# RobotSail/2048-PPO

Measured on AMD Instinct MI355X. Metric: env-steps/sec (whole node) at 65536 parallel 4x4 boards, 1/2/4/8 MI355X, higher is better.
Workload: dtype int8

## Files before the change

2048-ppo_amd/csrc/env_rollout.hip:

```cpp
#include <hip/hip_runtime.h>
#include <stdint.h>

#include <atomic>
#include <type_traits>

#include "board.hpp"
#include "rowtable.hpp"
#include "line11_lds.hpp"
#include "step.hpp"
#include "rollout_step.hpp"
#include "launch_util.hpp"
#include "../../include/g2048.h"

using namespace g2048;

namespace {

__device__ __forceinline__ uint4 fresh_from_words(const uint4 &r, uint32_t &p1, uint32_t &v1, uint32_t &p2,
                                                  uint32_t &v2) {
    p1 = r.x >> 28;
    v1 = r.y < kTwoThreshold ? 1u : 2u;
    const uint32_t k2 = (uint32_t)(((uint64_t)r.z * 15u) >> 32);
    p2 = k2 + (k2 >= p1 ? 1u : 0u);
    v2 = r.w < kTwoThreshold ? 1u : 2u;
// ... 42 lines not shown
template <int kAddr, bool kWide>
__global__ __launch_bounds__(1024) void env_rollout_kernel(uint4 *__restrict__ boards, int64_t n, int64_t steps,
                                                           uint4 *__restrict__ tb, uint8_t *__restrict__ ta,
                                                           int32_t *__restrict__ tp, uint32_t *__restrict__ tpot,
                                                           uint8_t *__restrict__ tf, RngArgs rng,
                                                           uint32_t *__restrict__ ticket) {
    __shared__ __attribute__((aligned(16))) uint32_t s_row[kRolloutLdsWords];
    i32x4 fa{};
    if constexpr (kAddr != kAddrValu) fa = line_mfma_frag();
    stage_row_table(s_row);
    if constexpr (kAddr != kAddrValu) asm volatile("" : "+v"(fa));
    const uint64_t ctr0 = rng_counter(rng);
    const int64_t stride = (int64_t)gridDim.x * blockDim.x;
    for (int64_t i = (int64_t)blockIdx.x * blockDim.x + threadIdx.x; i < n; i += stride) {
        RolloutLane s;
        s.b = boards[i];
        const uint32_t env = rng.env_base + (uint32_t)i;
        const uint32_t li = (uint32_t)i;
        s.legal = legal_mask(s.b);
        if (s.legal == 0u) {
            uint32_t p1, v1, p2, v2;
            s.b = fresh_from_words(philox_draw(rng.seed, ctr0 + (uint64_t)steps, env, 2u), p1, v1, p2, v2);
            MonoStats ms;
            s.legal = fresh_stats(p1, v1, p2, v2, ms);
            s.S = carry_pack(ms);
        } else {
            s.S = carry_pack(mono_stats(s.b));
        }
        s.empt_b = emptiness(s.b);
        uint64_t pair = ctr0 >> 1;
        s.D = philox_draw(rng.seed, pair, env, 1u);
        s.ph = philox_start(rng.seed, pair + 1u, env, 1u);
        fresh_prep(s, s_row);
        refill_lines<kAddr>(s, s_row, s.S >> 24, fa);
        using Rows = std::conditional_t<kWide, TrajRows, TrajRowsNarrow>;
        Rows tr = Rows::at(tb, ta, tp, tpot, tf, li);
        uint64_t left = (uint64_t)steps;
        if ((ctr0 & 1u) && left > 0u) {
            philox_rounds<0, 5>(s.ph);
            rollout_step<true, false, true, kAddr, Rows>(s, s_row, tr, rng.seed, pair + 2u, env, fa);
            tr.next(n);
            pair++;
            left--;
        }
        for (uint64_t pairs = left >> 1; pairs != 0u; pairs--, pair++) {
            if (__all(s.S < ((kFastPairMax + 1u) << 24))) {
                rollout_step<false, true, true, kAddr, Rows>(s, s_row, tr, rng.seed, pair + 2u, env, fa);
                tr.next(n);
                rollout_step<true, true, true, kAddr, Rows>(s, s_row, tr, rng.seed, pair + 2u, env, fa);
            } else {
                rollout_step<false, false, true, kAddr, Rows>(s, s_row, tr, rng.seed, pair + 2u, env, fa);
                tr.next(n);
                rollout_step<true, false, true, kAddr, Rows>(s, s_row, tr, rng.seed, pair + 2u, env, fa);
            }
            tr.next(n);
        }
        if (left & 1u) rollout_step<false, false, true, kAddr, Rows>(s, s_row, tr, rng.seed, pair + 2u, env, fa);
        boards[i] = s.b;
    }
    if (ticket) {
        __syncthreads();
        if (threadIdx.x == 0 &&
            __hip_atomic_fetch_add(ticket, 1u, __ATOMIC_RELAXED, __HIP_MEMORY_SCOPE_AGENT) == gridDim.x - 1u) {
            __hip_atomic_fetch_add(const_cast<uint64_t *>(rng.counter_dev), (uint64_t)steps, __ATOMIC_RELAXED,
                                   __HIP_MEMORY_SCOPE_AGENT);
            __hip_atomic_store(ticket, 0u, __ATOMIC_RELAXED, __HIP_MEMORY_SCOPE_AGENT);
        }
// ... 64 lines not shown
```

2048-ppo_amd/csrc/line11_lds.hpp:

```cpp
#pragma once
#include <hip/hip_runtime.h>
#include <stdint.h>

#include "board.hpp"
#include "rowtable.hpp"

namespace {

__device__ const g2048::lut::Line11Table kLine11 __attribute__((aligned(16))) = g2048::lut::Line11Table();
static_assert(g2048::lut::line11_table_ok(g2048::lut::Line11Table()), "kLine11 fields against slide_entry / line_entry");

__device__ const g2048::lut::FreshTable kFresh __attribute__((aligned(16))) = g2048::lut::FreshTable();
__device__ const g2048::lut::FreshLineTable kFreshLines __attribute__((aligned(16))) = g2048::lut::FreshLineTable();
static_assert(g2048::lut::fresh_lines_ok(g2048::lut::FreshTable(), g2048::lut::FreshLineTable()), "kFreshLines against the kFresh boards");
constexpr uint32_t kLineLdsBytes = g2048::lut::kFusedEntriesPadded * 8u;
constexpr uint32_t kFreshBoardBase = kLineLdsBytes;
constexpr uint32_t kFreshLineBase = kFreshBoardBase + g2048::lut::kFreshEntries * 16u;
constexpr uint32_t kFreshStatBase = kFreshLineBase + g2048::lut::kFreshEntries * 16u;
constexpr uint32_t kRolloutLdsWords = (kFreshStatBase + 4096u) / 4u;
static_assert(kRolloutLdsWords * 4u <= 160u * 1024u, "the tables fit the 160 KiB of LDS");
constexpr uint32_t kMaxLineDigit = g2048::lut::kLineBase - 1u;
static_assert(8u * g2048::lut::line11_index(kMaxLineDigit, kMaxLineDigit, kMaxLineDigit, kMaxLineDigit) + 8u <= g2048::lut::kFusedEntries * 8u &&
              g2048::lut::kFusedEntries * 8u <= kLineLdsBytes, "kLine11 reads stay inside the table");
static_assert(g2048::lut::line11_index(kMaxLineDigit, kMaxLineDigit, kMaxLineDigit, kMaxLineDigit) < 65536u, "column indices fit the packed-u16 sums");

typedef uint16_t u16x2 __attribute__((ext_vector_type(2)));
__device__ __forceinline__ u16x2 as_u16x2(uint32_t x) { return __builtin_bit_cast(u16x2, x); }

__device__ __forceinline__ void line11_addrs(const uint4 &b, uint32_t (&ra)[4], uint32_t (&ca)[4]) {
    const u16x2 k02 = {8, 968}, k13 = {88, 10648};
    const uint32_t w[4] = {b.x, b.y, b.z, b.w};
    u16x2 A[4], B[4];
#pragma unroll
    for (int i = 0; i < 4; i++) {
        A[i] = as_u16x2(__builtin_amdgcn_perm(0u, w[i], 0x0C020C00u));
        B[i] = as_u16x2(__builtin_amdgcn_perm(0u, w[i], 0x0C030C01u));
        ra[i] = __builtin_amdgcn_udot2(B[i], k13, __builtin_amdgcn_udot2(A[i], k02, 0u, false), false);
    }
    const u16x2 c02 = A[0] + A[1] * (u16x2){11, 11} + A[2] * (u16x2){121, 121} + A[3] * (u16x2){1331, 1331};
    const u16x2 c13 = B[0] + B[1] * (u16x2){11, 11} + B[2] * (u16x2){121, 121} + B[3] * (u16x2){1331, 1331};
    const uint32_t p02 = __builtin_bit_cast(uint32_t, c02), p13 = __builtin_bit_cast(uint32_t, c13);
    ca[0] = (p02 & 0xFFFFu) << 3;
    ca[1] = (p13 & 0xFFFFu) << 3;
    ca[2] = (p02 >> 16) << 3;
    ca[3] = (p13 >> 16) << 3;
}

typedef int i32x4 __attribute__((ext_vector_type(4)));
typedef int i32x16 __attribute__((ext_vector_type(16)));
constexpr uint32_t kLineHiScale = 8u * g2048::lut::kLineBase * g2048::lut::kLineBase;
constexpr int line_mfma_weight(uint32_t q, uint32_t c) {
    const uint32_t line = q & 7u, r = c >> 2, col = c & 3u;
    const uint32_t pos = line < 4u ? (r == line ? col : 4u) : (col == line - 4u ? r : 4u);
// ... 43 lines not shown
                const uint32_t lo_c = (uint32_t)line_mfma_model(t, h ? other : mine, h ? mine : other, h, 4u + r);
                const uint32_t hi_c = (uint32_t)line_mfma_model(t, h ? other : mine, h ? mine : other, h, 12u + r);
                if (lo_r > 960u || hi_r > 120u || lo_c > 960u || hi_c > 120u) return false;
                if (lo_r + kLineHiScale * hi_r != 8u * g2048::lut::line11_index(c[4 * r], c[4 * r + 1], c[4 * r + 2], c[4 * r + 3])) return false;
                if (lo_c + kLineHiScale * hi_c != 8u * g2048::lut::line11_index(c[r], c[4 + r], c[8 + r], c[12 + r])) return false;
            }
        }
    return true;
}
static_assert(line_mfma_weights_int8(), "the MFMA address weights fit int8");
static_assert(line_mfma_ok(), "the MFMA address model against line11_index");
__device__ const LineMfmaTable kLineMfmaA __attribute__((aligned(16))) = LineMfmaTable();
__device__ __forceinline__ i32x4 line_mfma_frag() {
    return *reinterpret_cast<const i32x4 *>(kLineMfmaA.a[threadIdx.x & 63u]);
}
__device__ __forceinline__ i32x16 line11_limbs_mfma(const uint4 &b, const i32x4 &fa) {
    const i32x4 bv = {(int)b.x, (int)b.y, (int)b.z, (int)b.w};
    const i32x16 zero = {0, 0, 0, 0, 0, 0, 0, 0, 0, 0, 0, 0, 0, 0, 0, 0};
    return __builtin_amdgcn_mfma_i32_32x32x32_i8(fa, bv, zero, 0, 0, 0);
}
__device__ __forceinline__ void line11_addrs_from_limbs(const i32x16 &d, uint32_t (&ra)[4], uint32_t (&ca)[4]) {
#pragma unroll
    for (int i = 0; i < 4; i++) {
        ra[i] = __umul24((uint32_t)d[8 + i], kLineHiScale) + (uint32_t)d[i];
        ca[i] = __umul24((uint32_t)d[12 + i], kLineHiScale) + (uint32_t)d[4 + i];
    }
}
__device__ __forceinline__ void line11_addrs_mfma(const uint4 &b, const i32x4 &fa, uint32_t (&ra)[4], uint32_t (&ca)[4]) {
    line11_addrs_from_limbs(line11_limbs_mfma(b, fa), ra, ca);
}
__device__ __forceinline__ uint2 lds_rec(const uint32_t *tab, uint32_t addr) {
    return *reinterpret_cast<const uint2 *>(reinterpret_cast<const char *>(tab) + addr);
}
__device__ __forceinline__ uint32_t lds_half(const uint32_t *tab, uint32_t addr) {
    return *reinterpret_cast<const uint16_t *>(reinterpret_cast<const char *>(tab) + addr);
}

constexpr uint32_t kUnpackStartSel = 0x05010400u;
constexpr uint32_t kUnpackEndSel = 0x07030602u;

constexpr uint32_t kPackRowsSel = 0x05040100u;
constexpr uint32_t kPackColsSel = 0x05010400u;
constexpr uint32_t kPackEndAdd = 0x02020202u;
constexpr uint32_t perm_model(uint32_t hi, uint32_t lo, uint32_t sel) {
    const uint64_t src = ((uint64_t)hi << 32) | lo;
    uint32_t r = 0u;
    for (uint32_t j = 0u; j < 4u; j++) {
        const uint32_t s = (sel >> (8u * j)) & 0xFFu;
        r |= (s < 8u ? (uint32_t)(src >> (8u * s)) & 0xFFu : 0u) << (8u * j);
    }
    return r;
}
struct Rows4 {
    uint32_t x, y, z, w;
};
constexpr Rows4 orient_rows_model(uint32_t e0, uint32_t e1, uint32_t e2, uint32_t e3, bool vert, bool rev) {
    const uint32_t psel = (vert ? kPackColsSel : kPackRowsSel) + (rev ? kPackEndAdd : 0u);
    const uint32_t x02 = perm_model(e2, e0, psel), x13 = perm_model(e3, e1, psel);
    const uint32_t xl02 = x02 & 0x0F0F0F0Fu, xh02 = (x02 >> 4) & 0x0F0F0F0Fu;
    const uint32_t xl13 = x13 & 0x0F0F0F0Fu, xh13 = (x13 >> 4) & 0x0F0F0F0Fu;
    const uint32_t pA = vert ? xl13 : xh02, pB = vert ? xh02 : xl13;
    return Rows4{perm_model(pA, xl02, kUnpackStartSel), perm_model(xh13, pB, kUnpackStartSel),
                 perm_model(pA, xl02, kUnpackEndSel), perm_model(xh13, pB, kUnpackEndSel)};
}
constexpr Rows4 unpack_transpose_model(uint32_t e0, uint32_t e1, uint32_t e2, uint32_t e3, bool vert, bool rev) {
    const uint32_t usel = rev ? kUnpackEndSel : kUnpackStartSel;
    const uint32_t w[4] = {perm_model(e0 >> 4, e0, usel) & 0x0F0F0F0Fu, perm_model(e1 >> 4, e1, usel) & 0x0F0F0F0Fu,
                           perm_model(e2 >> 4, e2, usel) & 0x0F0F0F0Fu, perm_model(e3 >> 4, e3, usel) & 0x0F0F0F0Fu};
    const uint32_t p = perm_model(w[1], w[0], 0x05010400u), q = perm_model(w[1], w[0], 0x07030602u);
    const uint32_t u = perm_model(w[3], w[2], 0x05010400u), v = perm_model(w[3], w[2], 0x07030602u);
    if (!vert) return Rows4{w[0], w[1], w[2], w[3]};
    return Rows4{perm_model(u, p, 0x05040100u), perm_model(u, p, 0x07060302u), perm_model(v, q, 0x05040100u),
                 perm_model(v, q, 0x07060302u)};
}
constexpr bool orient_rows_ok() {
    for (uint32_t k = 0u; k < 11u; k++) {
        uint32_t e[4] = {0u, 0u, 0u, 0u};
        for (uint32_t i = 0u; i < 4u; i++)
            for (uint32_t j = 0u; j < 8u; j++) e[i] |= ((k + 3u * j + 5u * i) % 11u) << (4u * j);
        for (uint32_t o = 0u; o < 4u; o++) {
            const Rows4 n = orient_rows_model(e[0], e[1], e[2], e[3], (o & 2u) != 0u, (o & 1u) != 0u);
            const Rows4 r = unpack_transpose_model(e[0], e[1], e[2], e[3], (o & 2u) != 0u, (o & 1u) != 0u);
            if (n.x != r.x || n.y != r.y || n.z != r.z || n.w != r.w) return false;
        }
    }
    return true;
}
static_assert(orient_rows_ok(), "the orientation network against unpack_row, transpose and sel4");
__device__ __forceinline__ uint4 orient_rows(uint32_t e0, uint32_t e1, uint32_t e2, uint32_t e3, uint32_t psel, bool vert) {
    const uint32_t x02 = __builtin_amdgcn_perm(e2, e0, psel), x13 = __builtin_amdgcn_perm(e3, e1, psel);
    const uint32_t xl02 = x02 & 0x0F0F0F0Fu, xh02 = (x02 >> 4) & 0x0F0F0F0Fu;
    const uint32_t xl13 = x13 & 0x0F0F0F0Fu, xh13 = (x13 >> 4) & 0x0F0F0F0Fu;
    const uint32_t pA = vert ? xl13 : xh02, pB = vert ? xh02 : xl13;
    return make_uint4(__builtin_amdgcn_perm(pA, xl02, kUnpackStartSel), __builtin_amdgcn_perm(xh13, pB, kUnpackStartSel),
                      __builtin_amdgcn_perm(pA, xl02, kUnpackEndSel), __builtin_amdgcn_perm(xh13, pB, kUnpackEndSel));
}

typedef __attribute__((address_space(3))) void lds_void_t;
typedef __attribute__((address_space(1))) void glb_void_t;
__device__ __forceinline__ void stage_row_table(uint32_t *s_row) {
    constexpr int kLinePieces = (int)(kLineLdsBytes / 1024u);
    constexpr int kFreshPieces = (int)(g2048::lut::kFreshEntries * 16u / 1024u);
    static_assert(kLineLdsBytes % 1024u == 0u && g2048::lut::kFreshEntries * 16u % 1024u == 0u, "whole 1 KiB pieces");
    static_assert(sizeof(kLine11.v) == kLineLdsBytes && sizeof(kFresh.b) == kFreshPieces * 1024 &&
                  sizeof(kFreshLines.a) == kFreshPieces * 1024 && sizeof(kFresh.st) == 4096, "table sizes");
    constexpr int kAll = kLinePieces + 2 * kFreshPieces + 4;
    static_assert(kAll * 1024 == (int)(kRolloutLdsWords * 4u), "the pieces fill the allocation");
    const char *src = reinterpret_cast<const char *>(kLine11.v);
    const char *src2 = reinterpret_cast<const char *>(kFresh.b);
    const char *src3 = reinterpret_cast<const char *>(kFreshLines.a);
    const char *src4 = reinterpret_cast<const char *>(kFresh.st);
    char *dst = reinterpret_cast<char *>(s_row);
    const int lane = threadIdx.x & 63, wave = threadIdx.x >> 6, nw = blockDim.x >> 6;
    for (int c = wave; c < kAll; c += nw) {
        const char *g;
        if (c < kLinePieces) g = src + 1024 * c;
        else if (c < kLinePieces + kFreshPieces) g = src2 + 1024 * (c - kLinePieces);
        else if (c < kLinePieces + 2 * kFreshPieces) g = src3 + 1024 * (c - kLinePieces - kFreshPieces);
        else g = src4 + 1024 * (c - kLinePieces - 2 * kFreshPieces);
        __builtin_amdgcn_global_load_lds((glb_void_t *)(g + 16 * lane), (lds_void_t *)(dst + 1024 * c), 16, 0, 0);
    }
    __builtin_amdgcn_s_waitcnt(0);
    __syncthreads();
}

}
```

2048-ppo_amd/csrc/mc_search.hip:

```cpp
#include <hip/hip_runtime.h>
#include <stdint.h>

#include "board.hpp"
#include "rowtable.hpp"
#include "line11_lds.hpp"
#include "step.hpp"
#include "rollout_step.hpp"
#include "launch_util.hpp"
#include "../../include/g2048.h"

using namespace g2048;

namespace {

constexpr int64_t kMaxPlayouts = 4096, kMaxDepth = 65536;

__device__ __forceinline__ void mc_playout(RolloutLane &s, const uint32_t *__restrict__ tab, uint64_t seed, uint64_t c,
                                           uint32_t env, int depth) {
    refill_lines(s, tab, s.M);
    const TrajRows none{};
    uint64_t pair = c >> 1;
    s.D = philox_draw(seed, pair, env, 1u);
    s.ph = philox_start(seed, pair + 1u, env, 1u);
    int t = 0;
    if (c & 1u) {
        philox_rounds<0, 5>(s.ph);
        rollout_step<true, false, false>(s, tab, none, seed, pair + 2u, env);
        pair++;
        t = 1;
    }
    for (; s.legal != 0u && t + 2 <= depth; t += 2, pair++) {
        if (__all(s.M <= kFastPairMax)) {
            rollout_step<false, true, false>(s, tab, none, seed, pair + 2u, env);
            if (s.legal == 0u) break;
            rollout_step<true, true, false>(s, tab, none, seed, pair + 2u, env);
        } else {
            rollout_step<false, false, false>(s, tab, none, seed, pair + 2u, env);
            if (s.legal == 0u) break;
            rollout_step<true, false, false>(s, tab, none, seed, pair + 2u, env);
        }
    }
    if (s.legal != 0u && t < depth) rollout_step<false, false, false>(s, tab, none, seed, pair + 2u, env);
}

__global__ __launch_bounds__(1024) void mc_search_kernel(const uint4 *__restrict__ boards, uint32_t total,
                                                         uint32_t playouts, int depth, RngArgs rng,
                                                         unsigned long long *__restrict__ score_sum,
                                                         unsigned long long *__restrict__ move_sum,
                                                         uint8_t *__restrict__ legal_out, uint8_t *__restrict__ best_out,
                                                         uint32_t *__restrict__ arrived) {
    __shared__ __attribute__((aligned(16))) uint32_t s_row[kRolloutLdsWords];
    stage_row_table(s_row);
    const uint64_t ctr0 = rng_counter(rng);
    const uint32_t lane = threadIdx.x & 63u;
    const uint32_t stride = gridDim.x * blockDim.x;
    for (uint32_t L0 = blockIdx.x * blockDim.x + (threadIdx.x & ~63u); L0 < total; L0 += stride) {
        const uint32_t L = L0 + lane;
        const bool valid = L < total;
        uint32_t g = 0xFFFFFFFFu, p = 0u;
        uint32_t score = 0u, moves = 0u;
        if (valid) {
            g = L / playouts;
            p = L - g * playouts;
            const uint4 root = boards[g >> 2];
            uint32_t pts0, mx0;
            uint4 moved = apply_move(root, g & 3u, pts0, mx0);
            if (!eq4(moved, root)) {
                const uint32_t env = rng.env_base + L;
                const uint4 ph = philox_draw(rng.seed, ctr0, env, 0u);
                spawn<G2048_RNG_PHILOX>(moved, ph.x, ph.y, nullptr, rng, (int64_t)L);
                RolloutLane s;
                s.b = moved;
                s.legal = legal_mask(moved);
                s.M = board_max(moved);
                s.score = pts0;
                s.moves = 0u;
                if (s.legal != 0u && depth > 0) mc_playout(s, s_row, rng.seed, ctr0, env, depth);
                score = s.score;
                moves = s.moves;
            }
        }
        unsigned long long sc = score;
        uint32_t mv = moves;
#pragma unroll
        for (uint32_t off = 1u; off < 64u; off <<= 1) {
// ... 85 lines not shown
```

2048-ppo_amd/csrc/rollout_step.hpp:

```cpp
#pragma once
#include <hip/hip_runtime.h>
#include <stdint.h>

#include "board.hpp"
#include "rowtable.hpp"
#include "line11_lds.hpp"
#include "step.hpp"

namespace {

using namespace g2048;

constexpr uint32_t kFastPairMax = 8u;
static_assert(kFastPairMax + 1u + 1u <= kMaxLineDigit, "a fast pair (start <= 8) stays inside kLine11");
static_assert(lut::kFreshLineAddrMax + 8u <= kLineLdsBytes, "fresh boards' line records inside kLine11");
static_assert(60u * 15u + 4u * 14u + 3u == lut::kFreshEntries - 1u, "kFresh index range");
static_assert(kFreshStatBase + 4u * lut::kFreshEntries <= kRolloutLdsWords * 4u, "kFresh reads stay inside the allocation");

__device__ __forceinline__ uint32_t mono_value_packed(uint32_t S) {
    const u16x2 m = __builtin_elementwise_max(as_u16x2(S & 0x000F0F00u), as_u16x2((S >> 4) & 0x000F0F00u));
    const uint32_t best256 = __builtin_amdgcn_udot2(m, (u16x2){1, 256}, 0u, false);
    const uint32_t corner = __builtin_amdgcn_ubfe(0x9009u, S, 1u);
    return best256 >> (9u - 2u * corner);
}
__device__ __forceinline__ uint32_t stats_bytes(uint32_t SR, uint32_t SC) {
    return __builtin_amdgcn_perm(SC, SR, 0x0C04000Cu);
}

struct RolloutLane {
    uint4 b;
    uint32_t legal;
    uint32_t M;
    uint32_t S;
    int empt_b;
    uint2 R[4], C[4];
    uint4 D;
    PhiloxState ph;
    uint32_t fbo;
    uint32_t fst;
    uint4 fla;
    uint32_t score;
    uint32_t moves;
};

__device__ __forceinline__ void fresh_prep(RolloutLane &s, const uint32_t *__restrict__ tab) {
    const uint32_t a = s.D.z, bw = s.D.w;
    const uint64_t pb = (uint64_t)bw * 15u;
    const uint32_t k2 = (uint32_t)(pb >> 32);
    const uint32_t i = 60u * (a >> 28) + 4u * k2 + ((a << 4) >= kTwoThreshold ? 2u : 0u) +
                       ((uint32_t)pb >= kTwoThreshold ? 1u : 0u);
    const char *t = reinterpret_cast<const char *>(tab);
    s.fbo = kFreshBoardBase + 16u * i;
    s.fla = *reinterpret_cast<const uint4 *>(t + kFreshLineBase + 16u * i);
    s.fst = *reinterpret_cast<const uint32_t *>(t + kFreshStatBase + 4u * i);
}
__device__ __forceinline__ void reset_reload(RolloutLane &s, const uint32_t *__restrict__ tab) {
    uint4 la = s.fla;
    asm volatile("" : "+v"(la.x), "+v"(la.y), "+v"(la.z), "+v"(la.w));
    s.b = *reinterpret_cast<const uint4 *>(reinterpret_cast<const char *>(tab) + s.fbo);
    s.R[0] = lds_rec(tab, la.x & 0xFFFFu);
    s.R[1] = lds_rec(tab, la.x >> 16);
    s.R[2] = lds_rec(tab, la.y & 0xFFFFu);
    s.R[3] = lds_rec(tab, la.y >> 16);
    s.C[0] = lds_rec(tab, la.z & 0xFFFFu);
    s.C[1] = lds_rec(tab, la.z >> 16);
    s.C[2] = lds_rec(tab, la.w & 0xFFFFu);
    s.C[3] = lds_rec(tab, la.w >> 16);
}

constexpr int kAddrValu = 0, kAddrMfma = 1;

template <int kAddr = kAddrValu>
__device__ __forceinline__ void refill_lines(RolloutLane &s, const uint32_t *__restrict__ tab, uint32_t mx, const i32x4 &fa = i32x4{}) {
    const uint4 ab = sel4(mx > kMaxLineDigit, make_uint4(0u, 0u, 0u, 0u), s.b);
    uint32_t ra[4], ca[4];
    if constexpr (kAddr == kAddrValu) line11_addrs(ab, ra, ca);
    else line11_addrs_mfma(ab, fa, ra, ca);
#pragma unroll
    for (int i = 0; i < 4; i++) {
        s.R[i] = lds_rec(tab, ra[i]);
        s.C[i] = lds_rec(tab, ca[i]);
    }
}

constexpr int kWaitLds = 0xC07F;

struct TrajRows {
    uint4 *b;
    uint8_t *a;
    int32_t *p;
    uint32_t *pot;
    uint8_t *f;
    __device__ __forceinline__ static TrajRows at(uint4 *tb, uint8_t *ta, int32_t *tp, uint32_t *tpot, uint8_t *tf, uint32_t i) {
        return TrajRows{tb + i, ta + i, tp + i, tpot + i, tf + i};
    }
    __device__ __forceinline__ void next(int64_t n) {
        b += n;
        a += n;
        p += n;
        pot += n;
        f += n;
    }
    __device__ __forceinline__ void put_b(const uint4 &v) const { *b = v; }
    __device__ __forceinline__ void put_a(uint32_t v) const { *a = (uint8_t)v; }
    __device__ __forceinline__ void put_p(uint32_t v) const { *p = (int32_t)v; }
    __device__ __forceinline__ void put_pot(uint32_t v) const { *pot = v; }
    __device__ __forceinline__ void put_f(uint32_t v) { *f = (uint8_t)v; }
};
struct TrajRowsNarrow {
    char *b, *a, *p, *pot, *f;
    uint32_t o1, o4, o16;
    __device__ __forceinline__ static TrajRowsNarrow at(uint4 *tb, uint8_t *ta, int32_t *tp, uint32_t *tpot, uint8_t *tf, uint32_t i) {
        return TrajRowsNarrow{(char *)tb, (char *)ta, (char *)tp, (char *)tpot, (char *)tf, i, 4u * i, 16u * i};
    }
    __device__ __forceinline__ void next(int64_t n) {
        const uint32_t n1 = (uint32_t)n;
        o1 += n1;
        o4 += 4u * n1;
        o16 += 16u * n1;
        asm("" : "+v"(o1), "+v"(o4), "+v"(o16));
    }
    __device__ __forceinline__ void put_b(const uint4 &v) const { *reinterpret_cast<uint4 *>(b + o16) = v; }
    __device__ __forceinline__ void put_a(uint32_t v) const { *reinterpret_cast<uint8_t *>(a + o1) = (uint8_t)v; }
    __device__ __forceinline__ void put_p(uint32_t v) const { *reinterpret_cast<int32_t *>(p + o4) = (int32_t)v; }
    __device__ __forceinline__ void put_pot(uint32_t v) const { *reinterpret_cast<uint32_t *>(pot + o4) = v; }
    __device__ __forceinline__ void put_f(uint32_t v) {
        asm("" : "+v"(o1));
        *reinterpret_cast<uint8_t *>(f + o1) = (uint8_t)v;
    }
};

template <bool kOdd, bool kSmall, bool kTraj, int kAddr = kAddrValu, class Rows = TrajRows>
__device__ __forceinline__ void rollout_step(RolloutLane &s, const uint32_t *__restrict__ tab, Rows &tr,
                                             uint64_t seed, uint64_t next_pair, uint32_t env, const i32x4 &fa = i32x4{}) {
    if constexpr (kTraj && (!kOdd || kSmall)) __builtin_amdgcn_s_waitcnt(kWaitLds);
    if constexpr (kTraj) tr.put_b(s.b);
    const uint32_t u = kOdd ? s.D.y : s.D.x;
    const uint64_t pa = (uint64_t)u * (uint32_t)__popc(s.legal);
    const uint32_t a = kth_bit4(s.legal, (uint32_t)(pa >> 32)), r = (uint32_t)pa;
    const bool vert = a < 2u, rev = (a & 1u) != 0u;
    const uint32_t e0 = vert ? s.C[0].x : s.R[0].x, e1 = vert ? s.C[1].x : s.R[1].x;
    const uint32_t e2 = vert ? s.C[2].x : s.R[2].x, e3 = vert ? s.C[3].x : s.R[3].x;
    const uint32_t h0 = vert ? s.C[0].y : s.R[0].y, h1 = vert ? s.C[1].y : s.R[1].y;
    const uint32_t h2 = vert ? s.C[2].y : s.R[2].y, h3 = vert ? s.C[3].y : s.R[3].y;
    const uint32_t mono_b = kTraj ? mono_value_packed(s.S) : 0u;
    const uint32_t pbase = vert ? kPackColsSel : kPackRowsSel;
    const uint32_t psel = rev ? pbase + kPackEndAdd : pbase;
    uint4 moved = orient_rows(e0, e1, e2, e3, psel, vert);
    uint32_t pts = (((h0 >> 16) & 0xFFFu) + ((h1 >> 16) & 0xFFFu) + ((h2 >> 16) & 0xFFFu) + ((h3 >> 16) & 0xFFFu)) << 2;
    uint32_t Ma = __builtin_bit_cast(uint32_t, __builtin_elementwise_max(__builtin_elementwise_max(as_u16x2(h0), as_u16x2(h1)),
                                                                         __builtin_elementwise_max(as_u16x2(h2), as_u16x2(h3)))) >> 28;
    if constexpr (kTraj && kSmall && !kOdd) __builtin_amdgcn_s_waitcnt(kWaitLds);
    if (!kSmall && (kTraj ? s.S >> 24 : s.M) > kMaxLineDigit) {
        uint32_t mx;
        moved = apply_move(s.b, a, pts, mx);
        Ma = board_max(moved);
    }
    const uint32_t rm[4] = {moved.x, moved.y, moved.z, moved.w};
    const uint32_t Zm[4] = {zm(moved.x), zm(moved.y), zm(moved.z), zm(moved.w)};
    uint32_t pos_a = 0u;
    if constexpr (kTraj && kAddr == kAddrValu) pos_a = first_cell_eq(rm, Ma);
    const uint32_t n0 = __popc(Zm[0]), n01 = __popc(Zm[1]) + n0, n012 = __popc(Zm[2]) + n01;
    const uint32_t empt_a = __popc(Zm[3]) + n012;
    const uint64_t prod = (uint64_t)r * empt_a;
    const uint32_t k = (uint32_t)(prod >> 32);
    const uint32_t v = (uint32_t)prod < kTwoThreshold ? 1u : 2u;
    const uint4 pre = moved;
    uint32_t row, col, mr0 = 0u, mr1 = 0u, mc0 = 0u, mc1 = 0u;
    bool r1 = false, r2 = false, r3 = false, c1 = false, c2 = false, c3 = false;
    if constexpr (kTraj) {
        const uint32_t P = n0 | (n01 << 8) | (n012 << 16);
        const uint32_t ger = (__umul24(k, 0x010101u) + (0x808080u - P)) & 0x808080u;
        row = __popc(ger);
        const uint32_t kr = k - __builtin_amdgcn_ubfe(P, 8u * row - 8u, 8u);
        mr0 = (uint32_t)__builtin_amdgcn_sbfe((int)row, 0u, 1u), mr1 = (uint32_t)__builtin_amdgcn_sbfe((int)ger, 15u, 1u);
        asm("" : "+v"(mr0), "+v"(mr1));
        const uint32_t z = pick4m(mr0, mr1, Zm[0], Zm[1], Zm[2], Zm[3]);
        const uint32_t PC = __umul24(z >> 7, 0x010101u);
        const uint32_t gec = (__umul24(kr, 0x010101u) + (0x808080u - PC)) & 0x808080u;
        col = __popc(gec);
        mc0 = (uint32_t)__builtin_amdgcn_sbfe((int)col, 0u, 1u), mc1 = (uint32_t)__builtin_amdgcn_sbfe((int)gec, 15u, 1u);
        asm("" : "+v"(mc0), "+v"(mc1));
        const uint32_t bits = v << (8u * col);
        const uint32_t blo = bop3<~kA & kB>(mr1, bits, 0u), bhi = mr1 & bits;
        moved.x = bop3<kA | (~kB & kC)>(moved.x, mr0, blo);
        moved.y = bop3<kA | (kB & kC)>(moved.y, mr0, blo);
// ... 25 lines not shown
    if constexpr (kAddr == kAddrValu) {
        line11_addrs(ab, ra, ca);
    } else {
        const i32x16 limbs = line11_limbs_mfma(ab, fa);
        if constexpr (kTraj) pos_a = first_cell_eq(rm, Ma);
        line11_addrs_from_limbs(limbs, ra, ca);
    }
    constexpr uint64_t kW11 = 0x299803C800580008ull;
    const uint32_t rq = kTraj ? pick4m(mr0, mr1, ra[0], ra[1], ra[2], ra[3]) : r3 ? ra[3] : r2 ? ra[2] : r1 ? ra[1] : ra[0];
    const uint32_t cq = kTraj ? pick4m(mc0, mc1, ca[0], ca[1], ca[2], ca[3]) : c3 ? ca[3] : c2 ? ca[2] : c1 ? ca[1] : ca[0];
    const uint32_t rp = rq - va * ((uint32_t)(kW11 >> (16u * col)) & 0xFFFFu);
    const uint32_t cp = cq - va * ((uint32_t)(kW11 >> (16u * row)) & 0xFFFFu);
    uint2 R0 = lds_rec(tab, ra[0]), R1 = lds_rec(tab, ra[1]), R2 = lds_rec(tab, ra[2]), R3 = lds_rec(tab, ra[3]);
    uint2 C0 = lds_rec(tab, ca[0]), C1 = lds_rec(tab, ca[1]), C2 = lds_rec(tab, ca[2]), C3 = lds_rec(tab, ca[3]);
    uint32_t fq = 0u, gq = 0u, fp = 0u, gp = 0u;
    if constexpr (kTraj) {
        fq = lds_half(tab, rq + 4u), gq = lds_half(tab, cq + 4u);
        fp = lds_half(tab, rp + 4u), gp = lds_half(tab, cp + 4u);
    }
    asm volatile("" : "+v"(s.ph.c0), "+v"(s.ph.c1), "+v"(s.ph.c2), "+v"(s.ph.c3)::"memory");
    if constexpr (kOdd) philox_rounds<5, 10>(s.ph);
    else philox_rounds<0, 5>(s.ph);
    if constexpr (kTraj)
        asm volatile("" : "+v"(s.ph.c0), "+v"(s.ph.c1), "+v"(s.ph.c2), "+v"(s.ph.c3), "+v"(R0.y), "+v"(R1.y), "+v"(R2.y), "+v"(R3.y),
                          "+v"(C0.y), "+v"(C1.y), "+v"(C2.y), "+v"(C3.y), "+v"(fq), "+v"(gq), "+v"(fp), "+v"(gp));
    else
        asm volatile("" : "+v"(s.ph.c0), "+v"(s.ph.c1), "+v"(s.ph.c2), "+v"(s.ph.c3), "+v"(R0.y), "+v"(R1.y), "+v"(R2.y), "+v"(R3.y),
                          "+v"(C0.y), "+v"(C1.y), "+v"(C2.y), "+v"(C3.y));
    if constexpr (kTraj) {
        tr.put_a(a);
        tr.put_p(pts);
    }
    const uint32_t SR = R0.y + R1.y + R2.y + R3.y, SC = C0.y + C1.y + C2.y + C3.y;
    const uint32_t SRp = SR - fq + fp, SCp = SC - gq + gp;
    const uint32_t nl = __builtin_amdgcn_perm(SR, SC, 0x0C0C0501u);
    s.legal = (__umul24((nl + 0x7777u) & 0x8888u, 0x249u) >> 12) & 15u;
    if (!kSmall && Ma > kMaxLineDigit) s.legal = legal_mask(moved);
    const bool over = s.legal == 0u;
    s.R[0] = R0, s.R[1] = R1, s.R[2] = R2, s.R[3] = R3;
    s.C[0] = C0, s.C[1] = C1, s.C[2] = C2, s.C[3] = C3;
    if constexpr (kTraj) {
        uint32_t sa = stats_bytes(SRp, SCp) | pos_a;
        const uint32_t pos2 = v > Ma ? sp : v == Ma ? min(pos_a, sp) : pos_a;
        uint32_t S = stats_bytes(SR, SC) | pos2 | (max(Ma, v) << 24);
        if (!kSmall && Ma > kMaxLineDigit) {
            const MonoStats ms = mono_stats(pre);
            sa = carry_pack(ms);
            S = carry_pack(mono_add_tile(ms, pre, sp, v));
        }
        const uint32_t mono_a = mono_value_packed(sa);
        tr.put_pot(mono_b | (mono_a << 8) | ((uint32_t)s.empt_b << 16) | (empt_a << 24));
        uint32_t fl = s.legal;
        s.S = S;
        s.empt_b = (int)empt_a - 1;
        if (over) {
            reset_reload(s, tab);
            uint32_t st = s.fst;
            asm volatile("" : "+v"(st));
            s.legal = st >> 28;
            s.S = st & 0x0FFFFFFFu;
            fl = FLAG_DONE | FLAG_RESET | s.legal;
            s.empt_b = 14;
        }
        tr.put_f(fl);
    } else {
        s.M = max(Ma, v);
        s.score += pts;
        s.moves += 1u;
    }
    if constexpr (kOdd) {
        s.D = make_uint4(s.ph.c0, s.ph.c1, s.ph.c2, s.ph.c3);
        s.ph = philox_start(seed, next_pair, env, 1u);
        if constexpr (kTraj) fresh_prep(s, tab);
    }
}

}
```

2048-ppo_amd/csrc/rowtable.hpp:

```cpp
#pragma once
#include <stdint.h>

namespace g2048 {
namespace lut {

constexpr uint32_t kRowBase = 12u;
constexpr uint32_t kRowEntries = kRowBase * kRowBase * kRowBase * kRowBase;

constexpr uint32_t slide_entry(uint32_t idx) {
    uint32_t c[4] = {idx % 12u, idx / 12u % 12u, idx / 144u % 12u, idx / 1728u};
    uint32_t nz[4] = {0u, 0u, 0u, 0u}, n = 0u;
    for (int j = 0; j < 4; j++)
        if (c[j]) nz[n++] = c[j];
    uint32_t out[4] = {0u, 0u, 0u, 0u}, m = 0u, i = 0u, pts = 0u;
    while (i < n) {
        if (i + 1u < n && nz[i] == nz[i + 1u]) {
            out[m++] = nz[i] + 1u;
            pts += 1u << (nz[i] + 1u);
            i += 2u;
        } else {
            out[m++] = nz[i];
            i += 1u;
        }
    }
// ... 8 lines not shown
        for (uint32_t i = 0; i < kRowEntries; i++) v[i] = slide_entry(i);
    }
};

constexpr uint32_t kLineEntriesPadded = 20992u;

constexpr uint16_t line_entry(uint32_t idx) {
    const uint32_t c[4] = {idx % 12u, idx / 12u % 12u, idx / 144u % 12u, idx / 1728u};
    uint32_t lc = 0u, rc = 0u, can0 = 0u, can3 = 0u;
    for (int j = 0; j < 3; j++) {
        const uint32_t a = c[j], b = c[j + 1];
        if (a != 0u && b != 0u) {
            lc += a >= b ? 1u : 0u;
            rc += b >= a ? 1u : 0u;
        }
        if ((a == 0u && b != 0u) || (a != 0u && a == b)) can0 = 1u;
        if ((a != 0u && b == 0u) || (a != 0u && a == b)) can3 = 1u;
    }
    return (uint16_t)(lc | (rc << 4) | (can0 << 8) | (can3 << 12));
}

struct Line12Table {
    uint16_t v[kLineEntriesPadded];
    constexpr Line12Table() : v() {
        for (uint32_t i = 0; i < kRowEntries; i++) v[i] = line_entry(i);
    }
};


constexpr uint32_t kFreshEntries = 16u * 15u * 4u;

struct FreshTable {
    uint32_t b[kFreshEntries * 4];
    uint32_t st[1024];
    constexpr FreshTable() : b(), st() {
        for (uint32_t p1 = 0; p1 < 16u; p1++)
            for (uint32_t k2 = 0; k2 < 15u; k2++)
                for (uint32_t w = 0; w < 4u; w++) {
                    const uint32_t i = 60u * p1 + 4u * k2 + w, p2 = k2 + (k2 >= p1 ? 1u : 0u);
                    const uint32_t v1 = 1u + (w >> 1), v2 = 1u + (w & 1u);
                    uint32_t c[16] = {};
                    c[p1] = v1;
                    c[p2] = v2;
                    for (uint32_t r = 0; r < 4u; r++)
                        b[4u * i + r] = c[4 * r] | (c[4 * r + 1] << 8) | (c[4 * r + 2] << 16) | (c[4 * r + 3] << 24);
                    uint32_t legal = 0u, L = 0u, R = 0u, T = 0u, B = 0u;
                    for (uint32_t r = 0; r < 4u; r++)
                        for (uint32_t j = 0; j < 3u; j++) {
                            const uint32_t x = c[4 * r + j], y = c[4 * r + j + 1];
                            const uint32_t u = c[4 * j + r], d = c[4 * j + 4 + r];
                            if ((x == 0u && y != 0u) || (x != 0u && x == y)) legal |= 4u;
                            if ((x != 0u && y == 0u) || (x != 0u && x == y)) legal |= 8u;
                            if ((u == 0u && d != 0u) || (u != 0u && u == d)) legal |= 1u;
                            if ((u != 0u && d == 0u) || (u != 0u && u == d)) legal |= 2u;
                            if (x != 0u && y != 0u) {
                                L += x >= y ? 1u : 0u;
                                R += y >= x ? 1u : 0u;
                            }
                            if (u != 0u && d != 0u) {
                                T += u >= d ? 1u : 0u;
                                B += d >= u ? 1u : 0u;
                            }
                        }
                    const uint32_t M = v1 > v2 ? v1 : v2;
                    uint32_t pos = 0u;
                    while (c[pos] != M) pos++;
                    st[i] = pos | (L << 8) | (R << 12) | (T << 16) | (B << 20) | (M << 24) | (legal << 28);
                }
    }
};

constexpr uint32_t kLineBase = 11u;
constexpr uint32_t kFusedEntries = kLineBase * kLineBase * kLineBase * kLineBase;
constexpr uint32_t kFusedEntriesPadded = 14720u;

constexpr uint32_t line11_index(uint32_t c0, uint32_t c1, uint32_t c2, uint32_t c3) {
    return c0 + 11u * c1 + 121u * c2 + 1331u * c3;
}
constexpr uint32_t row12_index(uint32_t c0, uint32_t c1, uint32_t c2, uint32_t c3) {
    return c0 + 12u * c1 + 144u * c2 + 1728u * c3;
}
constexpr uint32_t reverse_nibbles16(uint32_t x) {
    return ((x & 0xFu) << 12) | ((x & 0xF0u) << 4) | ((x >> 4) & 0xF0u) | ((x >> 12) & 0xFu);
}

struct Line11Table {
    uint32_t v[kFusedEntriesPadded * 2];
    constexpr Line11Table() : v() {
        for (uint32_t i = 0; i < kFusedEntries; i++) {
            const uint32_t c0 = i % 11u, c1 = i / 11u % 11u, c2 = i / 121u % 11u, c3 = i / 1331u;
            const uint32_t fwd = slide_entry(row12_index(c0, c1, c2, c3));
            const uint32_t bwd = slide_entry(row12_index(c3, c2, c1, c0));
            v[2u * i] = (fwd & 0xFFFFu) | (reverse_nibbles16(bwd & 0xFFFFu) << 16);
            v[2u * i + 1u] = line_entry(row12_index(c0, c1, c2, c3)) | (fwd & 0xFFFF0000u);
        }
    }
};

constexpr bool line11_table_ok(const Line11Table &t) {
    for (uint32_t i = 0; i < kFusedEntries; i++) {
// ... 17 lines not shown
static_assert(kFreshLineAddrMax < 65536u && kFreshLineAddrMax / 8u < kFusedEntries, "kFreshLines addresses");

struct FreshLineTable {
    uint16_t a[kFreshEntries * 8];
    constexpr FreshLineTable() : a() {
        for (uint32_t p1 = 0; p1 < 16u; p1++)
            for (uint32_t k2 = 0; k2 < 15u; k2++)
                for (uint32_t w = 0; w < 4u; w++) {
                    const uint32_t i = 60u * p1 + 4u * k2 + w, p2 = k2 + (k2 >= p1 ? 1u : 0u);
                    uint32_t c[16] = {};
                    c[p1] = 1u + (w >> 1);
                    c[p2] = 1u + (w & 1u);
                    for (uint32_t r = 0; r < 4u; r++) {
                        a[8u * i + r] = (uint16_t)(8u * line11_index(c[4 * r], c[4 * r + 1], c[4 * r + 2], c[4 * r + 3]));
                        a[8u * i + 4u + r] = (uint16_t)(8u * line11_index(c[r], c[4 + r], c[8 + r], c[12 + r]));
                    }
                }
    }
};

constexpr bool fresh_lines_ok(const FreshTable &f, const FreshLineTable &l) {
    for (uint32_t i = 0; i < kFreshEntries; i++) {
        uint32_t c[16] = {};
        for (uint32_t p = 0; p < 16u; p++) c[p] = (f.b[4u * i + p / 4u] >> (8u * (p % 4u))) & 0xFFu;
        for (uint32_t r = 0; r < 4u; r++) {
            if (l.a[8u * i + r] != 8u * line11_index(c[4 * r], c[4 * r + 1], c[4 * r + 2], c[4 * r + 3])) return false;
            if (l.a[8u * i + 4u + r] != 8u * line11_index(c[r], c[4 + r], c[8 + r], c[12 + r])) return false;
            if (l.a[8u * i + r] > kFreshLineAddrMax || l.a[8u * i + 4u + r] > kFreshLineAddrMax) return false;
        }
    }
    return true;
}

}
}
```

Before: 121.6 billion.

## Carry per-orientation line point sums and max in rollout lane state

In the trajectory rollout path, the per-row and per-column point sums and maxima of the line records' high words are now kept in lane state. They are computed once when lines are refilled or updated, instead of being rebuilt from four high words at each move. The high halves of R/C no longer need to be stored, and fresh-board resets load precomputed sums from an enlarged fresh stat table (8 bytes per entry). This costs extra LDS for the stat table and extra register state, and it tightens the large-tile fallback condition. It is meant to cut VALU work and register pressure per step.

After: 123.2 billion (median of 6 runs). 1.3% higher.

```diff
diff --git a/2048-ppo_amd/csrc/env_rollout.hip b/2048-ppo_amd/csrc/env_rollout.hip
--- a/2048-ppo_amd/csrc/env_rollout.hip
+++ b/2048-ppo_amd/csrc/env_rollout.hip
@@ -98,7 +98,7 @@
         s.D = philox_draw(rng.seed, pair, env, 1u);
         s.ph = philox_start(rng.seed, pair + 1u, env, 1u);
         fresh_prep(s, s_row);
-        refill_lines<kAddr>(s, s_row, s.S >> 24, fa);
+        refill_lines<kAddr, true>(s, s_row, s.S >> 24, fa);
         using Rows = std::conditional_t<kWide, TrajRows, TrajRowsNarrow>;
         Rows tr = Rows::at(tb, ta, tp, tpot, tf, li);
         uint64_t left = (uint64_t)steps;
diff --git a/2048-ppo_amd/csrc/line11_lds.hpp b/2048-ppo_amd/csrc/line11_lds.hpp
--- a/2048-ppo_amd/csrc/line11_lds.hpp
+++ b/2048-ppo_amd/csrc/line11_lds.hpp
@@ -13,12 +13,17 @@
 __device__ const g2048::lut::FreshTable kFresh __attribute__((aligned(16))) = g2048::lut::FreshTable();
 __device__ const g2048::lut::FreshLineTable kFreshLines __attribute__((aligned(16))) = g2048::lut::FreshLineTable();
 static_assert(g2048::lut::fresh_lines_ok(g2048::lut::FreshTable(), g2048::lut::FreshLineTable()), "kFreshLines against the kFresh boards");
+static_assert(g2048::lut::fresh_sums_ok(g2048::lut::FreshTable(), g2048::lut::FreshLineTable(), g2048::lut::Line11Table()),
+              "kFresh line sums against the kLine11 records of the kFresh boards");
 constexpr uint32_t kLineLdsBytes = g2048::lut::kFusedEntriesPadded * 8u;
 constexpr uint32_t kFreshBoardBase = kLineLdsBytes;
 constexpr uint32_t kFreshLineBase = kFreshBoardBase + g2048::lut::kFreshEntries * 16u;
 constexpr uint32_t kFreshStatBase = kFreshLineBase + g2048::lut::kFreshEntries * 16u;
-constexpr uint32_t kRolloutLdsWords = (kFreshStatBase + 4096u) / 4u;
+constexpr uint32_t kFreshStatPieces = 8u;
+constexpr uint32_t kRolloutLdsWords = (kFreshStatBase + 1024u * kFreshStatPieces) / 4u;
 static_assert(kRolloutLdsWords * 4u <= 160u * 1024u, "the tables fit the 160 KiB of LDS");
+constexpr uint32_t kSearchStatPieces = 4u;
+constexpr uint32_t kSearchLdsWords = (kFreshStatBase + 1024u * kSearchStatPieces) / 4u;
 constexpr uint32_t kMaxLineDigit = g2048::lut::kLineBase - 1u;
 static_assert(8u * g2048::lut::line11_index(kMaxLineDigit, kMaxLineDigit, kMaxLineDigit, kMaxLineDigit) + 8u <= g2048::lut::kFusedEntries * 8u &&
               g2048::lut::kFusedEntries * 8u <= kLineLdsBytes, "kLine11 reads stay inside the table");
@@ -128,6 +133,9 @@
 __device__ __forceinline__ uint2 lds_rec(const uint32_t *tab, uint32_t addr) {
     return *reinterpret_cast<const uint2 *>(reinterpret_cast<const char *>(tab) + addr);
 }
+__device__ __forceinline__ uint32_t lds_word(const uint32_t *tab, uint32_t addr) {
+    return *reinterpret_cast<const uint32_t *>(reinterpret_cast<const char *>(tab) + addr);
+}
 __device__ __forceinline__ uint32_t lds_half(const uint32_t *tab, uint32_t addr) {
     return *reinterpret_cast<const uint16_t *>(reinterpret_cast<const char *>(tab) + addr);
 }
@@ -194,14 +202,16 @@
 
 typedef __attribute__((address_space(3))) void lds_void_t;
 typedef __attribute__((address_space(1))) void glb_void_t;
+template <uint32_t kStatPieces = kFreshStatPieces>
 __device__ __forceinline__ void stage_row_table(uint32_t *s_row) {
     constexpr int kLinePieces = (int)(kLineLdsBytes / 1024u);
     constexpr int kFreshPieces = (int)(g2048::lut::kFreshEntries * 16u / 1024u);
     static_assert(kLineLdsBytes % 1024u == 0u && g2048::lut::kFreshEntries * 16u % 1024u == 0u, "whole 1 KiB pieces");
     static_assert(sizeof(kLine11.v) == kLineLdsBytes && sizeof(kFresh.b) == kFreshPieces * 1024 &&
-                  sizeof(kFreshLines.a) == kFreshPieces * 1024 && sizeof(kFresh.st) == 4096, "table sizes");
-    constexpr int kAll = kLinePieces + 2 * kFreshPieces + 4;
-    static_assert(kAll * 1024 == (int)(kRolloutLdsWords * 4u), "the pieces fill the allocation");
+                  sizeof(kFreshLines.a) == kFreshPieces * 1024 && sizeof(kFresh.st) == 1024u * kFreshStatPieces &&
+                  kStatPieces <= kFreshStatPieces, "table sizes");
+    constexpr int kAll = kLinePieces + 2 * kFreshPieces + (int)kStatPieces;
+    static_assert(kAll * 1024 == (int)(kFreshStatBase + 1024u * kStatPieces), "the pieces fill the allocation");
     const char *src = reinterpret_cast<const char *>(kLine11.v);
     const char *src2 = reinterpret_cast<const char *>(kFresh.b);
     const char *src3 = reinterpret_cast<const char *>(kFreshLines.a);
diff --git a/2048-ppo_amd/csrc/mc_search.hip b/2048-ppo_amd/csrc/mc_search.hip
--- a/2048-ppo_amd/csrc/mc_search.hip
+++ b/2048-ppo_amd/csrc/mc_search.hip
@@ -49,8 +49,8 @@
                                                          unsigned long long *__restrict__ move_sum,
                                                          uint8_t *__restrict__ legal_out, uint8_t *__restrict__ best_out,
                                                          uint32_t *__restrict__ arrived) {
-    __shared__ __attribute__((aligned(16))) uint32_t s_row[kRolloutLdsWords];
-    stage_row_table(s_row);
+    __shared__ __attribute__((aligned(16))) uint32_t s_row[kSearchLdsWords];
+    stage_row_table<kSearchStatPieces>(s_row);
     const uint64_t ctr0 = rng_counter(rng);
     const uint32_t lane = threadIdx.x & 63u;
     const uint32_t stride = gridDim.x * blockDim.x;
diff --git a/2048-ppo_amd/csrc/rollout_step.hpp b/2048-ppo_amd/csrc/rollout_step.hpp
--- a/2048-ppo_amd/csrc/rollout_step.hpp
+++ b/2048-ppo_amd/csrc/rollout_step.hpp
@@ -15,7 +15,11 @@
 static_assert(kFastPairMax + 1u + 1u <= kMaxLineDigit, "a fast pair (start <= 8) stays inside kLine11");
 static_assert(lut::kFreshLineAddrMax + 8u <= kLineLdsBytes, "fresh boards' line records inside kLine11");
 static_assert(60u * 15u + 4u * 14u + 3u == lut::kFreshEntries - 1u, "kFresh index range");
-static_assert(kFreshStatBase + 4u * lut::kFreshEntries <= kRolloutLdsWords * 4u, "kFresh reads stay inside the allocation");
+static_assert(kFreshStatBase + 8u * lut::kFreshEntries <= kRolloutLdsWords * 4u, "kFresh reads stay inside the allocation");
+
+constexpr uint32_t line_points4_max(uint32_t e) { return 4u * 2u * ((2u << e) >> 2); }
+static_assert(line_points4_max(kFastPairMax + 1u) < 4096u && line_points4_max(kMaxLineDigit - 1u) < 4096u &&
+              line_points4_max(kMaxLineDigit) == 4096u, "carried points sums stay inside their 12 bits");
 
 __device__ __forceinline__ uint32_t mono_value_packed(uint32_t S) {
     const u16x2 m = __builtin_elementwise_max(as_u16x2(S & 0x000F0F00u), as_u16x2((S >> 4) & 0x000F0F00u));
@@ -34,10 +38,12 @@
     uint32_t S;
     int empt_b;
     uint2 R[4], C[4];
+    uint32_t hsR, hsC;
+    uint32_t hmR, hmC;
     uint4 D;
     PhiloxState ph;
     uint32_t fbo;
-    uint32_t fst;
+    uint2 fst;
     uint4 fla;
     uint32_t score;
     uint32_t moves;
@@ -52,25 +58,25 @@
     const char *t = reinterpret_cast<const char *>(tab);
     s.fbo = kFreshBoardBase + 16u * i;
     s.fla = *reinterpret_cast<const uint4 *>(t + kFreshLineBase + 16u * i);
-    s.fst = *reinterpret_cast<const uint32_t *>(t + kFreshStatBase + 4u * i);
+    s.fst = *reinterpret_cast<const uint2 *>(t + kFreshStatBase + 8u * i);
 }
 __device__ __forceinline__ void reset_reload(RolloutLane &s, const uint32_t *__restrict__ tab) {
     uint4 la = s.fla;
     asm volatile("" : "+v"(la.x), "+v"(la.y), "+v"(la.z), "+v"(la.w));
     s.b = *reinterpret_cast<const uint4 *>(reinterpret_cast<const char *>(tab) + s.fbo);
-    s.R[0] = lds_rec(tab, la.x & 0xFFFFu);
-    s.R[1] = lds_rec(tab, la.x >> 16);
-    s.R[2] = lds_rec(tab, la.y & 0xFFFFu);
-    s.R[3] = lds_rec(tab, la.y >> 16);
-    s.C[0] = lds_rec(tab, la.z & 0xFFFFu);
-    s.C[1] = lds_rec(tab, la.z >> 16);
-    s.C[2] = lds_rec(tab, la.w & 0xFFFFu);
-    s.C[3] = lds_rec(tab, la.w >> 16);
+    s.R[0].x = lds_word(tab, la.x & 0xFFFFu);
+    s.R[1].x = lds_word(tab, la.x >> 16);
+    s.R[2].x = lds_word(tab, la.y & 0xFFFFu);
+    s.R[3].x = lds_word(tab, la.y >> 16);
+    s.C[0].x = lds_word(tab, la.z & 0xFFFFu);
+    s.C[1].x = lds_word(tab, la.z >> 16);
+    s.C[2].x = lds_word(tab, la.w & 0xFFFFu);
+    s.C[3].x = lds_word(tab, la.w >> 16);
 }
 
 constexpr int kAddrValu = 0, kAddrMfma = 1;
 
-template <int kAddr = kAddrValu>
+template <int kAddr = kAddrValu, bool kTraj = false>
 __device__ __forceinline__ void refill_lines(RolloutLane &s, const uint32_t *__restrict__ tab, uint32_t mx, const i32x4 &fa = i32x4{}) {
     const uint4 ab = sel4(mx > kMaxLineDigit, make_uint4(0u, 0u, 0u, 0u), s.b);
     uint32_t ra[4], ca[4];
@@ -80,6 +86,12 @@
     for (int i = 0; i < 4; i++) {
         s.R[i] = lds_rec(tab, ra[i]);
         s.C[i] = lds_rec(tab, ca[i]);
+    }
+    if constexpr (kTraj) {
+        s.hsR = s.R[0].y + s.R[1].y + s.R[2].y + s.R[3].y;
+        s.hsC = s.C[0].y + s.C[1].y + s.C[2].y + s.C[3].y;
+        s.hmR = max(max(s.R[0].y, s.R[1].y), max(s.R[2].y, s.R[3].y));
+        s.hmC = max(max(s.C[0].y, s.C[1].y), max(s.C[2].y, s.C[3].y));
     }
 }
 
@@ -141,17 +153,27 @@
     const bool vert = a < 2u, rev = (a & 1u) != 0u;
     const uint32_t e0 = vert ? s.C[0].x : s.R[0].x, e1 = vert ? s.C[1].x : s.R[1].x;
     const uint32_t e2 = vert ? s.C[2].x : s.R[2].x, e3 = vert ? s.C[3].x : s.R[3].x;
-    const uint32_t h0 = vert ? s.C[0].y : s.R[0].y, h1 = vert ? s.C[1].y : s.R[1].y;
-    const uint32_t h2 = vert ? s.C[2].y : s.R[2].y, h3 = vert ? s.C[3].y : s.R[3].y;
+    uint32_t h0 = 0u, h1 = 0u, h2 = 0u, h3 = 0u;
+    if constexpr (!kTraj) {
+        h0 = vert ? s.C[0].y : s.R[0].y, h1 = vert ? s.C[1].y : s.R[1].y;
+        h2 = vert ? s.C[2].y : s.R[2].y, h3 = vert ? s.C[3].y : s.R[3].y;
+    }
     const uint32_t mono_b = kTraj ? mono_value_packed(s.S) : 0u;
     const uint32_t pbase = vert ? kPackColsSel : kPackRowsSel;
     const uint32_t psel = rev ? pbase + kPackEndAdd : pbase;
     uint4 moved = orient_rows(e0, e1, e2, e3, psel, vert);
-    uint32_t pts = (((h0 >> 16) & 0xFFFu) + ((h1 >> 16) & 0xFFFu) + ((h2 >> 16) & 0xFFFu) + ((h3 >> 16) & 0xFFFu)) << 2;
-    uint32_t Ma = __builtin_bit_cast(uint32_t, __builtin_elementwise_max(__builtin_elementwise_max(as_u16x2(h0), as_u16x2(h1)),
-                                                                         __builtin_elementwise_max(as_u16x2(h2), as_u16x2(h3)))) >> 28;
+    uint32_t pts, Ma;
+    if constexpr (kTraj) {
+        const uint32_t hs = vert ? s.hsC : s.hsR, hm = vert ? s.hmC : s.hmR;
+        pts = (hs >> 14) & 0x3FFCu;
+        Ma = hm >> 28;
+    } else {
+        pts = (((h0 >> 16) & 0xFFFu) + ((h1 >> 16) & 0xFFFu) + ((h2 >> 16) & 0xFFFu) + ((h3 >> 16) & 0xFFFu)) << 2;
+        Ma = __builtin_bit_cast(uint32_t, __builtin_elementwise_max(__builtin_elementwise_max(as_u16x2(h0), as_u16x2(h1)),
+                                                                    __builtin_elementwise_max(as_u16x2(h2), as_u16x2(h3)))) >> 28;
+    }
     if constexpr (kTraj && kSmall && !kOdd) __builtin_amdgcn_s_waitcnt(kWaitLds);
-    if (!kSmall && (kTraj ? s.S >> 24 : s.M) > kMaxLineDigit) {
+    if (!kSmall && (kTraj ? (s.S >> 24) >= kMaxLineDigit : s.M > kMaxLineDigit)) {
         uint32_t mx;
         moved = apply_move(s.b, a, pts, mx);
         Ma = board_max(moved);
@@ -243,13 +265,23 @@
         tr.put_p(pts);
     }
     const uint32_t SR = R0.y + R1.y + R2.y + R3.y, SC = C0.y + C1.y + C2.y + C3.y;
+    if constexpr (kTraj) {
+        s.hsR = SR, s.hsC = SC;
+        s.hmR = max(max(R0.y, R1.y), max(R2.y, R3.y));
+        s.hmC = max(max(C0.y, C1.y), max(C2.y, C3.y));
+    }
     const uint32_t SRp = SR - fq + fp, SCp = SC - gq + gp;
     const uint32_t nl = __builtin_amdgcn_perm(SR, SC, 0x0C0C0501u);
     s.legal = (__umul24((nl + 0x7777u) & 0x8888u, 0x249u) >> 12) & 15u;
     if (!kSmall && Ma > kMaxLineDigit) s.legal = legal_mask(moved);
     const bool over = s.legal == 0u;
-    s.R[0] = R0, s.R[1] = R1, s.R[2] = R2, s.R[3] = R3;
-    s.C[0] = C0, s.C[1] = C1, s.C[2] = C2, s.C[3] = C3;
+    if constexpr (kTraj) {
+        s.R[0].x = R0.x, s.R[1].x = R1.x, s.R[2].x = R2.x, s.R[3].x = R3.x;
+        s.C[0].x = C0.x, s.C[1].x = C1.x, s.C[2].x = C2.x, s.C[3].x = C3.x;
+    } else {
+        s.R[0] = R0, s.R[1] = R1, s.R[2] = R2, s.R[3] = R3;
+        s.C[0] = C0, s.C[1] = C1, s.C[2] = C2, s.C[3] = C3;
+    }
     if constexpr (kTraj) {
         uint32_t sa = stats_bytes(SRp, SCp) | pos_a;
         const uint32_t pos2 = v > Ma ? sp : v == Ma ? min(pos_a, sp) : pos_a;
@@ -266,10 +298,12 @@
         s.empt_b = (int)empt_a - 1;
         if (over) {
             reset_reload(s, tab);
-            uint32_t st = s.fst;
-            asm volatile("" : "+v"(st));
+            uint32_t st = s.fst.x, hw = s.fst.y;
+            asm volatile("" : "+v"(st), "+v"(hw));
             s.legal = st >> 28;
             s.S = st & 0x0FFFFFFFu;
+            s.hsR = hw, s.hmR = hw;
+            s.hsC = hw << 16, s.hmC = hw << 16;
             fl = FLAG_DONE | FLAG_RESET | s.legal;
             s.empt_b = 14;
         }
diff --git a/2048-ppo_amd/csrc/rowtable.hpp b/2048-ppo_amd/csrc/rowtable.hpp
--- a/2048-ppo_amd/csrc/rowtable.hpp
+++ b/2048-ppo_amd/csrc/rowtable.hpp
@@ -64,7 +64,7 @@
 
 struct FreshTable {
     uint32_t b[kFreshEntries * 4];
-    uint32_t st[1024];
+    uint32_t st[2048];
     constexpr FreshTable() : b(), st() {
         for (uint32_t p1 = 0; p1 < 16u; p1++)
             for (uint32_t k2 = 0; k2 < 15u; k2++)
@@ -97,7 +97,11 @@
                     const uint32_t M = v1 > v2 ? v1 : v2;
                     uint32_t pos = 0u;
                     while (c[pos] != M) pos++;
-                    st[i] = pos | (L << 8) | (R << 12) | (T << 16) | (B << 20) | (M << 24) | (legal << 28);
+                    st[2u * i] = pos | (L << 8) | (R << 12) | (T << 16) | (B << 20) | (M << 24) | (legal << 28);
+                    const bool row_merge = p1 / 4u == p2 / 4u && v1 == v2, col_merge = p1 % 4u == p2 % 4u && v1 == v2;
+                    const uint32_t rows = ((row_merge ? v1 + 1u : M) << 12) | (row_merge ? (2u << v1) >> 2 : 0u);
+                    const uint32_t cols = ((col_merge ? v1 + 1u : M) << 12) | (col_merge ? (2u << v1) >> 2 : 0u);
+                    st[2u * i + 1u] = (rows << 16) | cols;
                 }
     }
 };
@@ -181,5 +185,24 @@
     return true;
 }
 
-}
-}
+constexpr bool fresh_sums_ok(const FreshTable &f, const FreshLineTable &l, const Line11Table &t) {
+    for (uint32_t i = 0; i < kFreshEntries; i++) {
+        uint32_t sum[2] = {0u, 0u}, mx[2] = {0u, 0u}, pts[2] = {0u, 0u};
+        for (uint32_t q = 0; q < 8u; q++) {
+            const uint32_t h = t.v[2u * (l.a[8u * i + q] / 8u) + 1u];
+            sum[q / 4u] += h;
+            mx[q / 4u] = h > mx[q / 4u] ? h : mx[q / 4u];
+            pts[q / 4u] += (h >> 16) & 0xFFFu;
+        }
+        const uint32_t w[2] = {f.st[2u * i + 1u], f.st[2u * i + 1u] << 16};
+        for (uint32_t o = 0; o < 2u; o++) {
+            if (pts[o] > 2u || (mx[o] >> 28) > 3u) return false;
+            if (((w[o] >> 16) & 0xFFFu) != ((sum[o] >> 16) & 0xFFFu) || ((sum[o] >> 16) & 0xFFFu) != pts[o]) return false;
+            if ((w[o] >> 28) != (mx[o] >> 28)) return false;
+        }
+    }
+    return true;
+}
+
+}
+}
```
